# Ezreal11/EaBNet

Hardware: AMD Instinct MI355X
Metric: enhanced frames/sec (16 kHz, 8-mic) at 1/2/4/8 MI355X; RTF per utterance (higher is better)
Workload: dtype f32; 1 GPU; BASELINE configs[1]/[2]: batch of 16 four-second 8-mic 16 kHz utterances per GPU, wave -> STFT+compress -> EaBNet.forward, inference, full hand-written HIP path; batch_per_gpu=16, global_batch=16, mics=8, frames_per_utt=401, freq_bins=161, parallelism=dp1 (independent shards, no collective), pipeline_depth=3

## Files before the change

### eabnet_amd/csrc/conv_gemm.hip

```cpp
#include "device.h"
#include <type_traits>

#define CG_THREADS 256

#define CG_PLAIN 0
#define CG_GLU 1
#define CG_DUAL 2
#define CG_PH2 3
#define CG_XFC 128

#define CG_PMAX 352

template <int MI, int NI, int KU, int MODE, bool PATCH, bool XFT>
struct CgSmem {
    static constexpr int BM = 64 * MI, BN = 64 * NI, LDK = 16 * KU + 4;
    static constexpr int NA = MODE == CG_DUAL ? 2 : 1;
    static constexpr int ATILE = BM * LDK;
    float a[PATCH ? CG_PMAX * LDK : NA * 2 * ATILE];
    float b[2][BN * LDK];
    float xft[2][CG_XFC][2];
    float xsl[2][CG_XFC];
    int dt[EAB_MAX_TAPS];
    int ioff[EAB_MAX_TAPS];
    int last;
    static constexpr int RW = MODE == CG_PH2 ? 2 : 1;
    __attribute__((aligned(16))) unsigned rtab_own[XFT ? BM * RW : 4];
    static_assert(XFT || sizeof(float) * 2 * CG_XFC * 2 >= sizeof(unsigned) * BM * RW, "row table inside xft");
};

__device__ __forceinline__ void cg_merge(float& n, float& mean, float& m2, float nb, float meanb, float m2b) {
    const float nt = n + nb;
    if (nt > 0.0f) {
        const float delta = meanb - mean;
        const float fb = nb / nt;
        mean = fmaf(delta, fb, mean);
        m2 = m2 + m2b + delta * delta * n * fb;
    }
    n = nt;
}

template <int MI, int NI, int KU, int MODE, int XF, bool VEC, int PREC, bool PATCH, bool WIDE = false>
__global__ __launch_bounds__(CG_THREADS, (MI == 2 && NI == 2 && KU == 1 && MODE == CG_GLU) ? 3 : (MODE == CG_PH2 ? 2 : 1)) void conv_gemm_kernel(const eab_conv_desc d) {
    static_assert(MODE != CG_PH2 || (PATCH && NI == 2), "phase-pair form: patch pipeline, one column block per phase and wave");
    static_assert(!PATCH || (KU == 1 && MODE != CG_DUAL && VEC), "patch mode: one unit per stage, single transform");
    constexpr bool H3 = PREC == EAB_PREC_F16X3;
    constexpr bool BF = PREC == EAB_PREC_BF16;
    constexpr bool PH2 = MODE == CG_PH2;
    constexpr bool GLU = MODE != CG_PLAIN;
    constexpr bool DUAL = MODE == CG_DUAL;
    using Smem = CgSmem<MI, NI, KU, MODE, PATCH, XF != EAB_XF_NONE>;
    constexpr int BM = Smem::BM, BN = Smem::BN, LDK = Smem::LDK;
    __shared__ __attribute__((aligned(16))) Smem sm;

    const int tid = threadIdx.x;
    const int lane = tid & 63, wave = tid >> 6;
    const int wm = wave >> 1, wn = wave & 1;
    const int li = lane & 31, lh = lane >> 5;

    const int t_lo = d.win.pos ? *d.win.pos : 0;
    int t_hi = d.win.pos ? (t_lo + d.win.count < d.T ? t_lo + d.win.count : d.T) : d.T;
    const int tiles_per_b = ((d.win.pos ? d.win.count : d.T) * d.No + BM - 1) / BM;
    unsigned vblk = blockIdx.x;
    if (gridDim.x >= 64) {
        const unsigned G = gridDim.x, G8 = G >> 3, rem = G & 7, xcd = vblk & 7, idx = vblk >> 3;
        vblk = xcd * G8 + (xcd < rem ? xcd : rem) + idx;
    }
    const int b = (int)(vblk / (unsigned)tiles_per_b);
    const int tile = (int)vblk - b * tiles_per_b;
    if (d.win.lens) t_hi = min(t_hi, d.win.lens[b]);
    const int Q = t_hi * d.No;
    const int q0 = t_lo * d.No + tile * BM;
    const int n_blk = blockIdx.y * BN;
    const float inv_no = 1.0f / (float)d.No;

#pragma unroll
    for (int j = 0; j < EAB_MAX_TAPS; ++j)
        if (tid == j) {
            sm.dt[j] = d.dt[j];
            sm.ioff[j] = d.ioff[j];
        }

    const int Cout = d.Cout;
    const unsigned row_bytes = (unsigned)(d.Fout * Cout) * 4u, step_bytes = (unsigned)(d.ostride * Cout) * 4u;
    const unsigned phase_bytes = (unsigned)(d.ophase * Cout) * 4u, chan_bytes = (unsigned)Cout * 4u;
    unsigned* const rtab = XF != EAB_XF_NONE ? sm.rtab_own : reinterpret_cast<unsigned*>(&sm.xft[0][0][0]);
    if (tid < BM) {
        const int q = q0 + tid;
        const bool ok = q < Q;
        const int t = eab_div(ok ? q : 0, d.No, inv_no), o = (ok ? q : 0) - t * d.No;
        const unsigned off = ok ? (unsigned)t * row_bytes + (unsigned)o * step_bytes + phase_bytes : EAB_OOB;
        if constexpr (PH2)
            *reinterpret_cast<uint2*>(&rtab[2 * tid]) = make_uint2(off, (ok && 2 * o + 1 < d.Fout) ? off + chan_bytes : EAB_OOB);
        else
            rtab[tid] = off;
    }

    if (XF != EAB_XF_NONE) {
        const int k = tid >> 7, c = tid & (CG_XFC - 1);
        const int Ck = (k == 0 || DUAL) ? d.C0 : d.C1;
        const float* xfk = k == 0 ? d.xf0 : d.xf1;
        const float* slk = k == 0 ? d.slope0 : d.slope1;
        float sc = 1.0f, sh = 0.0f, sl = 1.0f;
        if (c < Ck) {
            if (d.fin_stats && k < d.fin_nsets) {
                const float* gm = k == 0 ? d.fin_gamma0 : d.fin_gamma1;
                const float* bt = k == 0 ? d.fin_beta0 : d.fin_beta1;
                double sn = 0.0, sm = 0.0, sq = 0.0;
                for (int t = 0; t < d.fin_tiles; ++t) {
                    const f32x4 v = *reinterpret_cast<const f32x4*>(
                        &d.fin_stats[((((size_t)b * d.fin_tiles + t) * d.fin_nsets + k) * d.C0 + c) * 4]);
                    const double n = (double)v[0], mu = (double)v[1];
                    sn += n;
                    sm = fma(n, mu, sm);
                    sq += fma(n * mu, mu, (double)v[2]);
                }
                const double mean = sn > 0.0 ? sm / sn : 0.0;
                double var = sn > 0.0 ? sq / sn - mean * mean : 0.0;
                if (var < 0.0) var = 0.0;
                const double scale = (double)gm[c] / sqrt(var + (double)d.fin_eps);
                sc = (float)scale;
                sh = (float)((double)bt[c] - mean * scale);
                sl = slk[c];
            } else if (xfk) {
                const float2 v = *reinterpret_cast<const float2*>(&xfk[((size_t)b * Ck + c) * 2]);
                sc = v.x;
                sh = v.y;
                sl = slk[c];
            }
        }
        sm.xft[k][c][0] = sc;
        sm.xft[k][c][1] = sh;
        sm.xsl[k][c] = sl;
    }

    const int Ctot = d.C0 + d.C1;
    const int UPT = (Ctot + 15) >> 4;
    const int NU = d.ntaps * UPT;
    static_assert(!WIDE || (PREC == EAB_PREC_BF16 && KU == 1 && VEC && !PATCH && XF == EAB_XF_NONE && MODE != CG_DUAL), "WIDE: see above");
    constexpr bool w0 = WIDE, w1 = WIDE;
    const int NS = (w0 || w1) ? d.ntaps * ((w0 ? d.C0 >> 5 : (d.C0 + 15) >> 4) + (d.C1 > 0 ? (w1 ? d.C1 >> 5 : (d.C1 + 15) >> 4) : 0))
                              : (NU + KU - 1) / KU;

    constexpr unsigned esz0 = WIDE ? 2u : 4u, esz1 = WIDE ? 2u : 4u;
    const unsigned bytes0 = (unsigned)d.T * d.Fin * d.C0 * esz0;
    const unsigned bytes1 = (unsigned)d.T * d.Fin * d.C1 * esz1;
    const __amdgpu_buffer_rsrc_t rs0 = __builtin_amdgcn_make_buffer_rsrc(
        const_cast<char*>(reinterpret_cast<const char*>(d.src0)) + (size_t)b * bytes0, 0, bytes0, 0x00020000);
    const __amdgpu_buffer_rsrc_t rs1 = __builtin_amdgcn_make_buffer_rsrc(
        const_cast<char*>(reinterpret_cast<const char*>(d.src1 ? d.src1 : d.src0)) + (d.src1 ? (size_t)b * bytes1 : 0), 0,
        d.src1 ? bytes1 : 0u, 0x00020000);

    const int srow = tid >> 2;
    const int skq = tid & 3;
    const float* wrow[NI];
#pragma unroll
    for (int p = 0; p < NI; ++p) wrow[p] = d.w + (size_t)(n_blk + srow + 64 * p) * d.Kpad + skq * 4;

    f32x16 acc[MI][NI];
#pragma unroll
    for (int mi = 0; mi < MI; ++mi)
#pragma unroll
        for (int ni = 0; ni < NI; ++ni)
#pragma unroll
            for (int r = 0; r < 16; ++r) acc[mi][ni][r] = 0.0f;

    auto lds_barrier = [] { asm volatile("s_waitcnt lgkmcnt(0)\n\ts_barrier" ::: "memory"); };

    __syncthreads();

    if (q0 < Q) {
    if constexpr (PATCH) {
        constexpr int PP = (CG_PMAX + 63) / 64;
        int dt_min = 0, io_min = 0, io_max = 0;
#pragma unroll
        for (int j = 0; j < EAB_MAX_TAPS; ++j)
            if (j < d.ntaps) {
                dt_min = d.dt[j] < dt_min ? d.dt[j] : dt_min;
                io_min = d.ioff[j] < io_min ? d.ioff[j] : io_min;
                io_max = d.ioff[j] > io_max ? d.ioff[j] : io_max;
            }
        const int halo_lo = -io_min;
        const int hi_need = (d.No - 1) * d.istride + io_max - (d.Fin - 1);
        const int Fp = d.Fin + halo_lo + (hi_need > 0 ? hi_need : 0);
        const float inv_fp = 1.0f / (float)Fp;
        const int t_first = eab_div(q0, d.No, inv_no);
        const int t_last = eab_div((q0 + BM < Q ? q0 + BM : (Q > q0 ? Q : q0 + 1)) - 1, d.No, inv_no);
        const int P = (t_last - t_first + 1 - dt_min) * Fp;

        const int d64 = eab_div(64, Fp, inv_fp), m64 = 64 - d64 * Fp;
        int p_tf[PP];
        bool p_ok[PP], p_all[PP];
        {
            const int tr = eab_div(srow, Fp, inv_fp);
            int f = srow - tr * Fp, t_in = t_first + dt_min + tr;
            int tf = t_in * d.Fin + f - halo_lo;
#pragma unroll
            for (int pp = 0; pp < PP; ++pp) {
                p_ok[pp] = p_all[pp] = false;
                p_tf[pp] = 0;
                if (64 * pp < P) {
                    p_ok[pp] = srow + 64 * pp < P && (unsigned)t_in < (unsigned)d.T && (unsigned)(f - halo_lo) < (unsigned)d.Fin;
                    if (XF != EAB_XF_NONE) p_all[pp] = __builtin_amdgcn_ballot_w64(p_ok[pp]) == __builtin_amdgcn_ballot_w64(true);
                    p_tf[pp] = tf;
                    f += m64;
                    t_in += d64;
                    tf += d64 * d.Fin + m64;
                    if (f >= Fp) {
                        f -= Fp;
                        ++t_in;
                        tf += d.Fin - Fp;
                    }
                }
            }
        }
        int fa[MI];
#pragma unroll
        for (int mi = 0; mi < MI; ++mi) {
            int q = q0 + (wm * MI + mi) * 32 + li;
            q = q < Q ? q : (Q > q0 ? Q - 1 : q0);
            const int t = eab_div(q, d.No, inv_no), o = q - t * d.No;
            fa[mi] = ((t - t_first - dt_min) * Fp + o * d.istride + halo_lo) * LDK + 4 * lh;
        }
        const int b_base = (wn * NI * 32 + li) * LDK + 4 * lh;

        f32x4 rp[PP];
        f32x4 rbw0[NI], rbw1[NI];
        int p_tc = 0;
        auto patch_fetch = [&](int chunk) {
            const int c0 = chunk << 4;
            const bool second = (d.C1 > 0) && (c0 >= d.C0);
            const int Cs = second ? d.C1 : d.C0;
            const int c = (second ? c0 - d.C0 : c0) + skq * 4;
            const bool cok = c < Cs;
            p_tc = ((second ? 1 : 0) << 8) | (cok ? c : 0);
#pragma unroll
            for (int pp = 0; pp < PP; ++pp) {
                if (64 * pp >= P) continue;
                const unsigned off = (p_ok[pp] && cok) ? (unsigned)((p_tf[pp] * Cs + c) * 4) : EAB_OOB;
                const u32x4 v = second ? __builtin_amdgcn_raw_buffer_load_b128(rs1, off, 0, 0)
                                       : __builtin_amdgcn_raw_buffer_load_b128(rs0, off, 0, 0);
                rp[pp] = __builtin_bit_cast(f32x4, v);
            }
        };
        auto patch_stash = [&]() {
            f32x4 sh01, sh23, sl;
            if (XF != EAB_XF_NONE) {
                const int cc = p_tc & 0xFF, tb = p_tc >> 8;
                sh01 = *reinterpret_cast<const f32x4*>(&sm.xft[tb][cc][0]);
                sh23 = *reinterpret_cast<const f32x4*>(&sm.xft[tb][cc + 2][0]);
                sl = *reinterpret_cast<const f32x4*>(&sm.xsl[tb][cc]);
            }
#pragma unroll
            for (int pp = 0; pp < PP; ++pp) {
                const int pidx = srow + 64 * pp;
                if (pidx >= CG_PMAX) continue;
                if (64 * pp >= P) continue;
                f32x4 v = rp[pp];
                if (XF != EAB_XF_NONE) {
                    const f32x4 x = eab_xform<XF>(v, sh01, sh23, sl);
                    v = x;
                    if (!p_all[pp]) {
                        asm volatile("; rim" ::: "memory");
                        v = p_ok[pp] ? x : f32x4{0.f, 0.f, 0.f, 0.f};
                    }
                }
                float* arow = &sm.a[pidx * LDK];
                if (BF) {
                    *reinterpret_cast<uint2*>(reinterpret_cast<char*>(arow) + skq * 8) = make_uint2(eab_bf2(v[0], v[1]), eab_bf2(v[2], v[3]));
                } else if (H3) {
                    unsigned h01, l01, h23, l23;
                    eab_split2(v[0], v[1], h01, l01);
                    eab_split2(v[2], v[3], h23, l23);
                    *reinterpret_cast<uint2*>(reinterpret_cast<char*>(arow) + skq * 8) = make_uint2(h01, h23);
                    *reinterpret_cast<uint2*>(reinterpret_cast<char*>(arow) + 32 + skq * 8) = make_uint2(l01, l23);
                } else {
                    *reinterpret_cast<f32x4*>(arow + skq * 4) = v;
                }
            }
        };
        auto b_fetch = [&](int u, f32x4 (&rbw)[NI]) {
            const int uu = u < NU ? u : 0;
#pragma unroll
            for (int p = 0; p < NI; ++p) rbw[p] = *reinterpret_cast<const f32x4*>(wrow[p] + (size_t)uu * 16);
        };
        auto b_stash = [&](int buf, const f32x4 (&rbw)[NI]) {
#pragma unroll
            for (int p = 0; p < NI; ++p) {
                float* brow = &sm.b[buf][(srow + 64 * p) * LDK];
                if (BF) {
                    *reinterpret_cast<uint2*>(reinterpret_cast<char*>(brow) + skq * 8) =
                        make_uint2(eab_bf2(rbw[p][0], rbw[p][1]), eab_bf2(rbw[p][2], rbw[p][3]));
                } else if (H3) {
                    const u32x4 w = __builtin_bit_cast(u32x4, rbw[p]);
                    *reinterpret_cast<uint2*>(reinterpret_cast<char*>(brow) + skq * 8) = make_uint2(w[0], w[1]);
                    *reinterpret_cast<uint2*>(reinterpret_cast<char*>(brow) + 32 + skq * 8) = make_uint2(w[2], w[3]);
                } else {
                    *reinterpret_cast<f32x4*>(brow + skq * 4) = rbw[p];
                }
            }
        };
        auto pcompute_n = [&](int cur, int tap, auto ne_c) {
            constexpr int NE = decltype(ne_c)::value;
            const int toff = (sm.dt[tap] * Fp + sm.ioff[tap]) * LDK;
            if (BF) {
                bf16x8 ab[MI], bb[NE];
#pragma unroll
                for (int mi = 0; mi < MI; ++mi) ab[mi] = *reinterpret_cast<const bf16x8*>(&sm.a[fa[mi] + toff]);
#pragma unroll
                for (int ni = 0; ni < NE; ++ni) bb[ni] = *reinterpret_cast<const bf16x8*>(&sm.b[cur][b_base + ni * 32 * LDK]);
#pragma unroll
                for (int mi = 0; mi < MI; ++mi)
#pragma unroll
                    for (int ni = 0; ni < NE; ++ni)
                        acc[mi][ni] = __builtin_amdgcn_mfma_f32_32x32x16_bf16(ab[mi], bb[ni], acc[mi][ni], 0, 0, 0);
            } else if (H3) {
                h16x8 ah[MI], al[MI], bh[NE], bl[NE];
#pragma unroll
                for (int mi = 0; mi < MI; ++mi) {
                    const char* pa = reinterpret_cast<const char*>(&sm.a[fa[mi] + toff]);
                    ah[mi] = *reinterpret_cast<const h16x8*>(pa);
                    al[mi] = *reinterpret_cast<const h16x8*>(pa + 32);
                }
#pragma unroll
                for (int ni = 0; ni < NE; ++ni) {
                    const char* pb = reinterpret_cast<const char*>(&sm.b[cur][b_base + ni * 32 * LDK]);
                    bh[ni] = *reinterpret_cast<const h16x8*>(pb);
                    bl[ni] = *reinterpret_cast<const h16x8*>(pb + 32);
                }
#pragma unroll
                for (int mi = 0; mi < MI; ++mi)
#pragma unroll
                    for (int ni = 0; ni < NE; ++ni) {
                        acc[mi][ni] = __builtin_amdgcn_mfma_f32_32x32x16_f16(al[mi], bh[ni], acc[mi][ni], 0, 0, 0);
                        acc[mi][ni] = __builtin_amdgcn_mfma_f32_32x32x16_f16(ah[mi], bl[ni], acc[mi][ni], 0, 0, 0);
                        acc[mi][ni] = __builtin_amdgcn_mfma_f32_32x32x16_f16(ah[mi], bh[ni], acc[mi][ni], 0, 0, 0);
                    }
            } else {
#pragma unroll
                for (int g = 0; g < 2; ++g) {
                    f32x4 af[MI], bf[NE];
#pragma unroll
                    for (int mi = 0; mi < MI; ++mi) af[mi] = *reinterpret_cast<const f32x4*>(&sm.a[fa[mi] + toff + g * 8]);
#pragma unroll
                    for (int ni = 0; ni < NE; ++ni)
                        bf[ni] = *reinterpret_cast<const f32x4*>(&sm.b[cur][b_base + ni * 32 * LDK + g * 8]);
#pragma unroll
                    for (int k = 0; k < 4; ++k)
#pragma unroll
                        for (int mi = 0; mi < MI; ++mi)
#pragma unroll
                            for (int ni = 0; ni < NE; ++ni)
                                acc[mi][ni] = __builtin_amdgcn_mfma_f32_32x32x2f32(af[mi][k], bf[ni][k], acc[mi][ni], 0, 0, 0);
                }
            }
        };
        const unsigned p2mask = PH2 ? (unsigned)d.p2_mask1 : ~0u;
        auto pcompute = [&](int cur, int tap) {
            if (PH2 && !((p2mask >> tap) & 1u)) pcompute_n(cur, tap, std::integral_constant<int, 1>{});
            else pcompute_n(cur, tap, std::integral_constant<int, NI>{});
        };

        patch_fetch(0);
        b_fetch(0, rbw0);
        patch_stash();
        b_stash(0, rbw0);
        b_fetch(1, rbw0);
        b_fetch(2, rbw1);
        lds_barrier();
        const int pre = d.ntaps >= 3 ? d.ntaps - 3 : 0;
        int chunk = 0, tap = 0;
        auto stage = [&](int u, int cur, f32x4 (&rnext)[NI]) {
            if (tap == pre && chunk + 1 < UPT) patch_fetch(chunk + 1);
            pcompute(cur, tap);
            if (u + 1 < NU) b_stash(cur ^ 1, rnext);
            b_fetch(u + 3, rnext);
            if (tap == d.ntaps - 1 && chunk + 1 < UPT) {
                lds_barrier();
                patch_stash();
            }
            lds_barrier();
            if (++tap == d.ntaps) { tap = 0; ++chunk; }
        };
        for (int u = 0; u < NU; u += 2) {
            stage(u, 0, rbw0);
            if (u + 1 < NU) stage(u + 1, 1, rbw1);
        }
        __syncthreads();
    } else {
    int a_t[MI], a_f0[MI], a_tf[MI];
    bool a_ok[MI];
#pragma unroll
    for (int p = 0; p < MI; ++p) {
        const int q = q0 + srow + 64 * p;
        a_ok[p] = q < Q;
        const int t = a_ok[p] ? eab_div(q, d.No, inv_no) : 0;
        const int o = a_ok[p] ? q - t * d.No : 0;
        a_t[p] = t;
        a_f0[p] = o * d.istride;
        a_tf[p] = t * d.Fin + o * d.istride;
    }
    struct Stage {
        f32x4 ra[KU][MI], rb[KU][NI];
        f32x4 rb2[BF ? NI : 1];
        int r_tc[KU];
        bool st_ok[KU][MI];
    };
    Stage sa;

    bool tap_ok[MI];
    unsigned tap_b0[MI], tap_b1[MI];
#pragma unroll
    for (int p = 0; p < MI; ++p) {
        tap_ok[p] = false;
        tap_b0[p] = tap_b1[p] = 0u;
    }
    int g_tap = -1, g_c0 = 0, g_w = 16;
    constexpr bool LEAN = KU == 1 && VEC && !DUAL;
    const __amdgpu_buffer_rsrc_t rsw = __builtin_amdgcn_make_buffer_rsrc(const_cast<float*>(d.w), 0, (unsigned)d.N * d.Kpad * 4u, 0x00020000);
// ... 121 lines not shown
                    const int tb = (rg.r_tc[ku] >> 8) & 1, cu = rg.r_tc[ku] & 0xFF;
                    const char* px = reinterpret_cast<const char*>(&sm.xft[0][skq * 4][0]) + (tb * CG_XFC + cu) * 8;
                    const char* ps = reinterpret_cast<const char*>(&sm.xsl[0][skq * 4]) + (tb * CG_XFC + cu) * 4;
                    sh01[0] = *reinterpret_cast<const f32x4*>(px);
                    sh23[0] = *reinterpret_cast<const f32x4*>(px + 16);
                    sl[0] = *reinterpret_cast<const f32x4*>(ps);
                    bool ok_all = true;
#pragma unroll
                    for (int p = 0; p < MI; ++p) ok_all = ok_all && rg.st_ok[ku][p];
                    all_ok = __builtin_amdgcn_ballot_w64(ok_all) == __builtin_amdgcn_ballot_w64(true);
                } else {
                const int cc = rg.r_tc[ku] & 0xFF;
#pragma unroll
                for (int k = 0; k < (DUAL ? 2 : 1); ++k) {
                    const int tb = DUAL ? k : (rg.r_tc[ku] >> 8);
                    sh01[k] = *reinterpret_cast<const f32x4*>(&sm.xft[tb][cc][0]);
                    sh23[k] = *reinterpret_cast<const f32x4*>(&sm.xft[tb][cc + 2][0]);
                    sl[k] = *reinterpret_cast<const f32x4*>(&sm.xsl[tb][cc]);
                }
                }
            }
#pragma unroll
            for (int p = 0; p < MI; ++p) {
#pragma unroll
                for (int k = 0; k < (DUAL ? 2 : 1); ++k) {
                    f32x4 v = rg.ra[ku][p];
                    if (XF != EAB_XF_NONE) {
                        v = eab_xform<XF>(v, sh01[k], sh23[k], sl[k]);
                        if (!all_ok) {
                            asm volatile("; rim" ::: "memory");
                            v = rg.st_ok[ku][p] ? v : f32x4{0.f, 0.f, 0.f, 0.f};
                        }
                    }
                    float* arow = &sm.a[(k * 2 + buf) * Smem::ATILE + (srow + 64 * p) * LDK + ku * 16];
                    if (BF) {
                        constexpr bool half = WIDE;
                        if (half)
                            *reinterpret_cast<u32x4*>(reinterpret_cast<char*>(arow) + skq * 16) = __builtin_bit_cast(u32x4, v);
                        else
                            *reinterpret_cast<uint2*>(reinterpret_cast<char*>(arow) + skq * 8) = make_uint2(eab_bf2(v[0], v[1]), eab_bf2(v[2], v[3]));
                    } else if (H3) {
                        unsigned h01, l01, h23, l23;
                        eab_split2(v[0], v[1], h01, l01);
                        eab_split2(v[2], v[3], h23, l23);
                        *reinterpret_cast<uint2*>(reinterpret_cast<char*>(arow) + skq * 8) = make_uint2(h01, h23);
                        *reinterpret_cast<uint2*>(reinterpret_cast<char*>(arow) + 32 + skq * 8) = make_uint2(l01, l23);
                    } else {
                        *reinterpret_cast<f32x4*>(arow + skq * 4) = v;
                    }
                }
            }
#pragma unroll
            for (int p = 0; p < NI; ++p) {
                float* brow = &sm.b[buf][(srow + 64 * p) * LDK + ku * 16];
                if (BF) {
                    if constexpr (WIDE) {
                        const f32x4 r0 = rg.rb[ku][p], r1 = rg.rb2[BF ? p : 0];
                        *reinterpret_cast<u32x4*>(reinterpret_cast<char*>(brow) + skq * 16) =
                            u32x4{eab_bf2(r0[0], r0[1]), eab_bf2(r0[2], r0[3]), eab_bf2(r1[0], r1[1]), eab_bf2(r1[2], r1[3])};
                    } else {
                        *reinterpret_cast<uint2*>(reinterpret_cast<char*>(brow) + skq * 8) =
                            make_uint2(eab_bf2(rg.rb[ku][p][0], rg.rb[ku][p][1]), eab_bf2(rg.rb[ku][p][2], rg.rb[ku][p][3]));
                    }
                } else if (H3) {
                    const u32x4 w = __builtin_bit_cast(u32x4, rg.rb[ku][p]);
                    *reinterpret_cast<uint2*>(reinterpret_cast<char*>(brow) + skq * 8) = make_uint2(w[0], w[1]);
                    *reinterpret_cast<uint2*>(reinterpret_cast<char*>(brow) + 32 + skq * 8) = make_uint2(w[2], w[3]);
                } else {
                    *reinterpret_cast<f32x4*>(brow + skq * 4) = rg.rb[ku][p];
                }
            }
        }
    };

    fetch(0, sa);
    stash(0, sa);
    lds_barrier();

    const int a_base = (wm * MI * 32 + li) * LDK + 4 * lh;
    const int b_base = (wn * NI * 32 + li) * LDK + 4 * lh;

    auto compute = [&](int cur) {
        if (BF) {
#pragma unroll
            for (int ku = 0; ku < KU; ++ku) {
                bf16x8 ab[Smem::NA][MI], bb[NI];
#pragma unroll
                for (int k = 0; k < Smem::NA; ++k)
#pragma unroll
                    for (int mi = 0; mi < MI; ++mi)
                        ab[k][mi] = *reinterpret_cast<const bf16x8*>(&sm.a[(k * 2 + cur) * Smem::ATILE + a_base + mi * 32 * LDK + ku * 16]);
#pragma unroll
                for (int ni = 0; ni < NI; ++ni) bb[ni] = *reinterpret_cast<const bf16x8*>(&sm.b[cur][b_base + ni * 32 * LDK + ku * 16]);
#pragma unroll
                for (int mi = 0; mi < MI; ++mi)
#pragma unroll
                    for (int ni = 0; ni < NI; ++ni)
                        acc[mi][ni] = __builtin_amdgcn_mfma_f32_32x32x16_bf16(ab[DUAL ? ni : 0][mi], bb[ni], acc[mi][ni], 0, 0, 0);
            }
            if constexpr (WIDE) {
                bf16x8 ab[MI], bb[NI];
#pragma unroll
                for (int mi = 0; mi < MI; ++mi) ab[mi] = *reinterpret_cast<const bf16x8*>(&sm.a[cur * Smem::ATILE + a_base + mi * 32 * LDK + 8]);
#pragma unroll
                for (int ni = 0; ni < NI; ++ni) bb[ni] = *reinterpret_cast<const bf16x8*>(&sm.b[cur][b_base + ni * 32 * LDK + 8]);
#pragma unroll
                for (int mi = 0; mi < MI; ++mi)
#pragma unroll
                    for (int ni = 0; ni < NI; ++ni)
                        acc[mi][ni] = __builtin_amdgcn_mfma_f32_32x32x16_bf16(ab[mi], bb[ni], acc[mi][ni], 0, 0, 0);
            }
        } else if (H3) {
#pragma unroll
            for (int ku = 0; ku < KU; ++ku) {
                h16x8 ah[Smem::NA][MI], al[Smem::NA][MI], bh[NI], bl[NI];
#pragma unroll
                for (int k = 0; k < Smem::NA; ++k)
#pragma unroll
                    for (int mi = 0; mi < MI; ++mi) {
                        const char* pa = reinterpret_cast<const char*>(&sm.a[(k * 2 + cur) * Smem::ATILE + a_base + mi * 32 * LDK + ku * 16]);
                        ah[k][mi] = *reinterpret_cast<const h16x8*>(pa);
                        al[k][mi] = *reinterpret_cast<const h16x8*>(pa + 32);
                    }
#pragma unroll
                for (int ni = 0; ni < NI; ++ni) {
                    const char* pb = reinterpret_cast<const char*>(&sm.b[cur][b_base + ni * 32 * LDK + ku * 16]);
                    bh[ni] = *reinterpret_cast<const h16x8*>(pb);
                    bl[ni] = *reinterpret_cast<const h16x8*>(pb + 32);
                }
#pragma unroll
                for (int mi = 0; mi < MI; ++mi)
#pragma unroll
                    for (int ni = 0; ni < NI; ++ni) {
                        const int ka = DUAL ? ni : 0;
                        acc[mi][ni] = __builtin_amdgcn_mfma_f32_32x32x16_f16(al[ka][mi], bh[ni], acc[mi][ni], 0, 0, 0);
                        acc[mi][ni] = __builtin_amdgcn_mfma_f32_32x32x16_f16(ah[ka][mi], bl[ni], acc[mi][ni], 0, 0, 0);
                        acc[mi][ni] = __builtin_amdgcn_mfma_f32_32x32x16_f16(ah[ka][mi], bh[ni], acc[mi][ni], 0, 0, 0);
                    }
            }
        } else {
#pragma unroll
        for (int g = 0; g < 2 * KU; ++g) {
            f32x4 af[Smem::NA][MI], bf[NI];
#pragma unroll
            for (int k = 0; k < Smem::NA; ++k)
#pragma unroll
                for (int mi = 0; mi < MI; ++mi)
                    af[k][mi] = *reinterpret_cast<const f32x4*>(&sm.a[(k * 2 + cur) * Smem::ATILE + a_base + mi * 32 * LDK + g * 8]);
#pragma unroll
            for (int ni = 0; ni < NI; ++ni)
                bf[ni] = *reinterpret_cast<const f32x4*>(&sm.b[cur][b_base + ni * 32 * LDK + g * 8]);
#pragma unroll
            for (int k = 0; k < 4; ++k)
#pragma unroll
                for (int mi = 0; mi < MI; ++mi)
#pragma unroll
                    for (int ni = 0; ni < NI; ++ni)
                        acc[mi][ni] = __builtin_amdgcn_mfma_f32_32x32x2f32(af[DUAL ? ni : 0][mi][k], bf[ni][k],
                                                                           acc[mi][ni], 0, 0, 0);
        }
        }
    };
    constexpr bool PF2 = MI * NI <= 2 && KU == 1 && MODE == CG_PLAIN;
    if constexpr (PF2) {
        Stage sb;
        if (NS > 1) fetch(1, sb);
        for (int s = 0; s < NS; s += 2) {
            if (s + 2 < NS) fetch(s + 2, sa);
            compute(0);
            if (s + 1 < NS) stash(1, sb);
            lds_barrier();
            if (s + 1 < NS) {
                if (s + 3 < NS) fetch(s + 3, sb);
                compute(1);
                if (s + 2 < NS) stash(0, sa);
                lds_barrier();
            }
        }
    } else {
    for (int s = 0; s < NS; ++s) {
        const int cur = s & 1;
// ... 210 lines not shown
                    }
                } else {
                    v = acc[mi][c][r] + bias_v[c];
                }
                if (d.epi == EAB_EPI_RELU) v = fmaxf(v, 0.0f);
                else if (d.epi == EAB_EPI_MULSIG) v = auxv[r][c] * eab_fast_sigmoid(v);
                else if (d.epi == EAB_EPI_ADD) v = v + auxv[r][c];
                const unsigned o4 = off[r] + 4u * ch[c];
                __builtin_amdgcn_raw_buffer_store_b32(__builtin_bit_cast(unsigned, v), r_dst, o4, 0, 0);
                if (d.dst_acc)
                    __builtin_amdgcn_raw_buffer_store_b32(__builtin_bit_cast(unsigned, v + accv[r][c]), r_acc, o4, 0, 0);
                if (rowok[r]) {
                    const bool first = scount == 0.0f;
                    const float g0 = eab_prelu(v, st_slope[0][c]);
                    if (first) skk[0][c] = g0;
                    const float e0 = g0 - skk[0][c];
                    ssum[0][c] += e0;
                    ssq[0][c] = fmaf(e0, e0, ssq[0][c]);
                    if (two_sets) {
                        const float g1 = eab_prelu(v, st_slope[1][c]);
                        if (first) skk[1][c] = g1;
                        const float e1 = g1 - skk[1][c];
                        ssum[1][c] += e1;
                        ssq[1][c] = fmaf(e1, e1, ssq[1][c]);
                    }
                }
            }
            if (rowok[r]) scount += 1.0f;
        }
    }

    }
    if (d.stats) {
        float* red = &sm.a[0];
        float mean[2][NC], m2[2][NC];
        float cnt = scount;
        const float inv_n = scount > 0.0f ? 1.0f / scount : 0.0f;
#pragma unroll
        for (int s = 0; s < 2; ++s)
#pragma unroll
            for (int c = 0; c < NC; ++c) {
                mean[s][c] = fmaf(ssum[s][c], inv_n, skk[s][c]);
                m2[s][c] = fmaxf(ssq[s][c] - ssum[s][c] * ssum[s][c] * inv_n, 0.0f);
            }
        const float cnt_o = __shfl_xor(cnt, 32);
#pragma unroll
        for (int s = 0; s < 2; ++s)
#pragma unroll
            for (int c = 0; c < NC; ++c) {
                float n = cnt;
                const float mo = __shfl_xor(mean[s][c], 32), qo = __shfl_xor(m2[s][c], 32);
                if (lh == 0) cg_merge(n, mean[s][c], m2[s][c], cnt_o, mo, qo);
            }
        cnt += cnt_o;
        if (lh == 0) {
#pragma unroll
            for (int s = 0; s < 2; ++s)
#pragma unroll
                for (int c = 0; c < NC; ++c) {
                    const int i = ((((wm * 2 + wn) * 2 + s) * NC + c) * 32 + li) * 3;
                    red[i] = cnt;
                    red[i + 1] = mean[s][c];
                    red[i + 2] = m2[s][c];
                }
        }
        __syncthreads();
        if (wm == 0 && lh == 0) {
            const size_t tbase = ((size_t)b * d.stat_tiles + d.stat_tile0 + tile) * d.nsets;
#pragma unroll
            for (int s = 0; s < 2; ++s) {
                if (s >= d.nsets) break;
#pragma unroll
                for (int c = 0; c < NC; ++c) {
                    const int i0 = ((((0 * 2 + wn) * 2 + s) * NC + c) * 32 + li) * 3;
                    const int i1 = ((((1 * 2 + wn) * 2 + s) * NC + c) * 32 + li) * 3;
                    float n = red[i0], mu = red[i0 + 1], q = red[i0 + 2];
                    cg_merge(n, mu, q, red[i1], red[i1 + 1], red[i1 + 2]);
                    *reinterpret_cast<f32x4*>(&d.stats[((tbase + s) * Cout + ch[c]) * 4]) = f32x4{n, mu, q, 0.0f};
                }
            }
        }
        if (d.fz_counter) {
            __threadfence();
            __syncthreads();
            if (tid == 0) sm.last = atomicAdd(&d.fz_counter[b], 1) == d.stat_tiles - 1;
            __syncthreads();
            if (sm.last) {
                __threadfence();
                const int nch = d.nsets * Cout;
                const int NSL = CG_THREADS / nch;
                const int e = tid % nch, slice = tid / nch;
                const int s = e / Cout, c = e - s * Cout;
                double* dred = reinterpret_cast<double*>(&sm.a[0]);
                double sn = 0.0, sm_ = 0.0, sq = 0.0;
                if (slice < NSL) {
                    const float* p = d.stats + (((size_t)b * d.stat_tiles) * d.nsets + s) * Cout * 4 + (size_t)c * 4;
                    const size_t stride = (size_t)d.nsets * Cout * 4;
                    for (int t = slice; t < d.stat_tiles; t += NSL) {
                        const f32x4 v = *reinterpret_cast<const f32x4*>(p + (size_t)t * stride);
                        const double n = (double)v[0], mu = (double)v[1];
                        sn += n;
                        sm_ = fma(n, mu, sm_);
                        sq += fma(n * mu, mu, (double)v[2]);
                    }
                    dred[(0 * NSL + slice) * nch + e] = sn;
                    dred[(1 * NSL + slice) * nch + e] = sm_;
                    dred[(2 * NSL + slice) * nch + e] = sq;
                }
                __syncthreads();
                if (slice == 0) {
                    sn = sm_ = sq = 0.0;
                    for (int k = 0; k < NSL; ++k) {
                        sn += dred[(0 * NSL + k) * nch + e];
                        sm_ += dred[(1 * NSL + k) * nch + e];
                        sq += dred[(2 * NSL + k) * nch + e];
                    }
                    const double mean = sn > 0.0 ? sm_ / sn : 0.0;
                    double var = sn > 0.0 ? sq / sn - mean * mean : 0.0;
                    if (var < 0.0) var = 0.0;
                    const float* gm = s == 0 ? d.fz_gamma0 : d.fz_gamma1;
                    const float* bt = s == 0 ? d.fz_beta0 : d.fz_beta1;
                    float* xf = s == 0 ? d.fz_xf0 : d.fz_xf1;
                    const double scale = (double)gm[c] / sqrt(var + (double)d.fz_eps);
                    *reinterpret_cast<float2*>(&xf[((size_t)b * Cout + c) * 2]) = make_float2((float)scale, (float)((double)bt[c] - mean * scale));
                }
                if (tid == 0) d.fz_counter[b] = 0;
// ... 2 lines not shown
    }
}

extern "C" int eab_conv_tiles(int T, int No, int bm) {
    if (T <= 0 || No <= 0 || (bm != 16 && bm != 32 && bm != 64 && bm != 128)) return -1;
    long long q = (long long)T * No;
    return (int)((q + bm - 1) / bm);
}

int eab_conv_st(const eab_conv_desc* d, hipStream_t s);

template <int MI, int NI, int KU, int MODE, int XF, bool VEC>
static int cg_launch(const eab_conv_desc* d, hipStream_t s) {
    constexpr int BM = 64 * MI, BN = 64 * NI;
    const int tiles = eab_conv_tiles(d->win.pos ? d->win.count : d->T, d->No, BM);
    dim3 grid((unsigned)(d->B * tiles), (unsigned)(d->N / BN));
    constexpr bool can_patch = KU == 1 && MODE != CG_DUAL && VEC && XF != EAB_XF_PRELU_NORM;
    if (d->korder == EAB_KORDER_CHUNK) {
        if constexpr (can_patch) {
            if (d->precision == EAB_PREC_F16X3)
                hipLaunchKernelGGL((conv_gemm_kernel<MI, NI, 1, MODE, XF, true, EAB_PREC_F16X3, true>), grid,
                                   dim3(CG_THREADS), 0, s, *d);
            else if (d->precision == EAB_PREC_BF16)
                hipLaunchKernelGGL((conv_gemm_kernel<MI, NI, 1, MODE, XF, true, EAB_PREC_BF16, true>), grid,
                                   dim3(CG_THREADS), 0, s, *d);
            else
                hipLaunchKernelGGL((conv_gemm_kernel<MI, NI, 1, MODE, XF, true, EAB_PREC_F32, true>), grid,
                                   dim3(CG_THREADS), 0, s, *d);
            EAB_RETURN_LAUNCH_STATUS();
        } else {
            return EAB_EUNSUPPORTED;
        }
    }
    if constexpr (MODE == CG_PH2) {
        return EAB_EUNSUPPORTED;
    } else {
    if (d->precision == EAB_PREC_F16X3) {
        if constexpr (VEC)
            hipLaunchKernelGGL((conv_gemm_kernel<MI, NI, KU, MODE, XF, VEC, EAB_PREC_F16X3, false>), grid,
                               dim3(CG_THREADS), 0, s, *d);
        else
            return EAB_EUNSUPPORTED;
    } else if (d->precision == EAB_PREC_BF16) {
        if constexpr (VEC) {
            if (d->src_bf16) {
                if constexpr (KU == 1 && XF == EAB_XF_NONE && MODE != CG_DUAL)
                    hipLaunchKernelGGL((conv_gemm_kernel<MI, NI, KU, MODE, XF, VEC, EAB_PREC_BF16, false, true>), grid,
                                       dim3(CG_THREADS), 0, s, *d);
                else
                    return EAB_EUNSUPPORTED;
            } else {
                hipLaunchKernelGGL((conv_gemm_kernel<MI, NI, KU, MODE, XF, VEC, EAB_PREC_BF16, false>), grid,
                                   dim3(CG_THREADS), 0, s, *d);
            }
        } else {
            return EAB_EUNSUPPORTED;
        }
    } else {
        hipLaunchKernelGGL((conv_gemm_kernel<MI, NI, KU, MODE, XF, VEC, EAB_PREC_F32, false>), grid, dim3(CG_THREADS), 0,
                           s, *d);
    }
    EAB_RETURN_LAUNCH_STATUS();
    }
}

static long long cg_patch_positions(const eab_conv_desc* d) {
    int dt_min = 0, io_min = 0, io_max = 0;
// ... 81 lines not shown
        EAB_CHECK_ARG(fin || (d->xf0 == nullptr) == (d->slope0 == nullptr));
        EAB_CHECK_ARG(fin || dual || (d->xf1 == nullptr) == (d->slope1 == nullptr));
    }
    if (dual) {
        EAB_CHECK_ARG(d->C1 == 0 && d->xf_mode != EAB_XF_NONE && d->slope0 && d->slope1);
        EAB_CHECK_ARG(fin || (d->xf0 && d->xf1));
    }
    EAB_CHECK_ARG((d->epi != EAB_EPI_MULSIG && d->epi != EAB_EPI_ADD) || d->aux);
    EAB_CHECK_ARG(d->nsets >= 0 && d->nsets <= 2 && (d->nsets == 0) == (d->stats == nullptr));
    EAB_CHECK_ARG(d->korder == EAB_KORDER_FRAG ? (d->bm == 16 || d->bm == 32 || d->bm == 64) : (d->bm == 64 || d->bm == 128));
    if (d->fz_counter) {
        EAB_CHECK_ARG(d->stats && d->nsets >= 1 && d->nsets * d->Cout <= CG_THREADS && d->win.pos == nullptr);
        EAB_CHECK_ARG(d->fz_gamma0 && d->fz_beta0 && d->fz_xf0 && (d->nsets == 1 || (d->fz_gamma1 && d->fz_beta1 && d->fz_xf1)));
    }
    if (d->stats) {
        const int tiles = eab_conv_tiles(d->T, d->No, d->bm) + (d->ph1_No > 0 ? eab_conv_tiles(d->T, d->ph1_No, d->bm) : 0);
        EAB_CHECK_ARG(d->stat_tile0 >= 0 && d->stat_tile0 + tiles <= d->stat_tiles);
    }
    EAB_CHECK_ARG((long long)d->B * (eab_conv_tiles(d->T, d->No, d->bm) + (d->ph1_No > 0 ? eab_conv_tiles(d->T, d->ph1_No, d->bm) : 0)) < (1ll << 31));
    hipStream_t s = eab_stream(stream);
    if (d->korder == EAB_KORDER_FRAG) return eab_conv_st(d, s);
    const int mi = d->bm / 64;
    const bool vec = (d->C0 % 4 == 0) && (d->C1 % 4 == 0);
    const bool has_xf = d->xf_mode != EAB_XF_NONE && (d->xf0 || d->xf1 || fin);
    const int xf = has_xf ? d->xf_mode : EAB_XF_NONE;
    if (xf != EAB_XF_NONE)
        EAB_CHECK_ARG(d->C0 <= CG_XFC && d->C1 <= CG_XFC && vec);
    int ku = (mi == 1 && !glu && vec && d->Fin == 1) ? 4 : 1;
    if (d->korder == EAB_KORDER_CHUNK) ku = 1;
    if (ku == 4 && !(mi == 1 && !glu && vec)) ku = 1;
    if (ku == 2 && (!vec || dual)) ku = 1;
    if (ph2) {
        if (!vec || xf == EAB_XF_PRELU_NORM) return EAB_EUNSUPPORTED;
        if (xf == EAB_XF_NORM_PRELU)
            return mi == 2 ? cg_launch<2, 2, 1, CG_PH2, EAB_XF_NORM_PRELU, true>(d, s) : cg_launch<1, 2, 1, CG_PH2, EAB_XF_NORM_PRELU, true>(d, s);
        return mi == 2 ? cg_launch<2, 2, 1, CG_PH2, EAB_XF_NONE, true>(d, s) : cg_launch<1, 2, 1, CG_PH2, EAB_XF_NONE, true>(d, s);
    }
    if (dual) {
        if (d->N != 128 || mi != 1 || xf != EAB_XF_PRELU_NORM) return EAB_EUNSUPPORTED;
        return cg_pick_ku<1, 2, CG_DUAL, EAB_XF_PRELU_NORM, true>(d, s, ku == 2 ? 1 : ku);
    }
    if (glu) {
        if (d->N % 128 != 0 || xf == EAB_XF_PRELU_NORM) return EAB_EUNSUPPORTED;
        if (!vec) return mi == 2 ? cg_pick_ku<2, 2, CG_GLU, 0, false>(d, s, 1) : cg_pick_ku<1, 2, CG_GLU, 0, false>(d, s, 1);
        if (xf == EAB_XF_NORM_PRELU)
            return mi == 2 ? cg_pick_ku<2, 2, CG_GLU, EAB_XF_NORM_PRELU, true>(d, s, ku)
                           : cg_pick_ku<1, 2, CG_GLU, EAB_XF_NORM_PRELU, true>(d, s, ku);
        return mi == 2 ? cg_pick_ku<2, 2, CG_GLU, 0, true>(d, s, ku) : cg_pick_ku<1, 2, CG_GLU, 0, true>(d, s, ku);
    }
    if (!vec) return EAB_EUNSUPPORTED;
#define CG_DISPATCH_XF(MI_, NI_)                                                           \
    (xf == EAB_XF_NONE        ? cg_pick_ku<MI_, NI_, CG_PLAIN, EAB_XF_NONE, true>(d, s, ku) \
     : xf == EAB_XF_NORM_PRELU ? cg_pick_ku<MI_, NI_, CG_PLAIN, EAB_XF_NORM_PRELU, true>(d, s, ku) \
                               : cg_pick_ku<MI_, NI_, CG_PLAIN, EAB_XF_PRELU_NORM, true>(d, s, ku))
    if (d->N % 128 == 0) return mi == 2 ? CG_DISPATCH_XF(2, 2) : CG_DISPATCH_XF(1, 2);
    if (d->N % 64 == 0) return mi == 2 ? CG_DISPATCH_XF(2, 1) : CG_DISPATCH_XF(1, 1);
#undef CG_DISPATCH_XF
    return EAB_EUNSUPPORTED;
}

extern "C" int eab_conv_bf16(const eab_conv_desc* d, eab_stream_t stream) {
    EAB_CHECK_ARG(d);
    eab_conv_desc dd = *d;
    dd.precision = EAB_PREC_BF16;
    return eab_conv_f32(&dd, stream);
}
// ... 1 lines not shown
```

Before: 997,500 frames/s.

## Double-buffer patch tile in phase-pair conv GEMM for two-tap layers

Adds a second LDS patch buffer for the phase-pair (PH2) patch pipeline. When a layer has exactly two taps, the next channel chunk is fetched and stashed into the alternate buffer while the current one is consumed, which removes the extra barrier that previously sat before each patch restash. It also defers building the norm/PReLU transform tables until after the first global loads are issued, so their latency overlaps. Other tap counts, or EAB_PATCH_BUFS=1, fall back to a single-buffer PH2S variant. The cost is doubled patch LDS, which is held under a static assert so two workgroups still fit per CU.

```diff
diff --git a/eabnet_amd/csrc/conv_gemm.hip b/eabnet_amd/csrc/conv_gemm.hip
--- a/eabnet_amd/csrc/conv_gemm.hip
+++ b/eabnet_amd/csrc/conv_gemm.hip
@@ -1,4 +1,5 @@
 #include "device.h"
+#include <cstdlib>
 #include <type_traits>
 
 #define CG_THREADS 256
@@ -7,23 +8,26 @@
 #define CG_GLU 1
 #define CG_DUAL 2
 #define CG_PH2 3
+#define CG_PH2S 4
 #define CG_XFC 128
 
 #define CG_PMAX 352
+#define CG_LDS_CU 163840
 
 template <int MI, int NI, int KU, int MODE, bool PATCH, bool XFT>
 struct CgSmem {
     static constexpr int BM = 64 * MI, BN = 64 * NI, LDK = 16 * KU + 4;
     static constexpr int NA = MODE == CG_DUAL ? 2 : 1;
     static constexpr int ATILE = BM * LDK;
-    float a[PATCH ? CG_PMAX * LDK : NA * 2 * ATILE];
+    static constexpr int PBUF = (PATCH && MODE == CG_PH2) ? 2 : 1;
+    float a[PBUF][PATCH ? CG_PMAX * LDK : NA * 2 * ATILE];
     float b[2][BN * LDK];
     float xft[2][CG_XFC][2];
     float xsl[2][CG_XFC];
     int dt[EAB_MAX_TAPS];
     int ioff[EAB_MAX_TAPS];
     int last;
-    static constexpr int RW = MODE == CG_PH2 ? 2 : 1;
+    static constexpr int RW = (MODE == CG_PH2 || MODE == CG_PH2S) ? 2 : 1;
     __attribute__((aligned(16))) unsigned rtab_own[XFT ? BM * RW : 4];
     static_assert(XFT || sizeof(float) * 2 * CG_XFC * 2 >= sizeof(unsigned) * BM * RW, "row table inside xft");
 };
@@ -39,17 +43,62 @@
     n = nt;
 }
 
+#define CG_XF_TABLES()                                                                                                         \
+    if (XF != EAB_XF_NONE) {                                                                                                   \
+                                          \
+                                           \
+                                             \
+                                                                \
+        const int k = tid >> 7, c = tid & (CG_XFC - 1);                                                                        \
+        const int Ck = (k == 0 || DUAL) ? d.C0 : d.C1;                                                                         \
+        const float* xfk = k == 0 ? d.xf0 : d.xf1;                                                                             \
+        const float* slk = k == 0 ? d.slope0 : d.slope1;                                                                       \
+        float sc = 1.0f, sh = 0.0f, sl = 1.0f;                                                                                 \
+        if (c < Ck) {                                                                                                          \
+            if (d.fin_stats && k < d.fin_nsets) {                                                                              \
+                const float* gm = k == 0 ? d.fin_gamma0 : d.fin_gamma1;                                                        \
+                const float* bt = k == 0 ? d.fin_beta0 : d.fin_beta1;                                                          \
+                double sn = 0.0, sm = 0.0, sq = 0.0;                               \
+                for (int t = 0; t < d.fin_tiles; ++t) {                                                                        \
+                    const f32x4 v = *reinterpret_cast<const f32x4*>(                                                           \
+                        &d.fin_stats[((((size_t)b * d.fin_tiles + t) * d.fin_nsets + k) * d.C0 + c) * 4]);                     \
+                    const double n = (double)v[0], mu = (double)v[1];                                                          \
+                    sn += n;                                                                                                   \
+                    sm = fma(n, mu, sm);                                                                                       \
+                    sq += fma(n * mu, mu, (double)v[2]);                                                                       \
+                }                                                                                                              \
+                const double mean = sn > 0.0 ? sm / sn : 0.0;                                                                  \
+                double var = sn > 0.0 ? sq / sn - mean * mean : 0.0;                                                           \
+                if (var < 0.0) var = 0.0;                                                                                      \
+                const double scale = (double)gm[c] / sqrt(var + (double)d.fin_eps);                                            \
+                sc = (float)scale;                                                                                             \
+                sh = (float)((double)bt[c] - mean * scale);                                                                    \
+                sl = slk[c];                                                                                                   \
+            } else if (xfk) {                                                                                                  \
+                const float2 v = *reinterpret_cast<const float2*>(&xfk[((size_t)b * Ck + c) * 2]);                             \
+                sc = v.x;                                                                                                      \
+                sh = v.y;                                                                                                      \
+                sl = slk[c];                                                                                                   \
+            }                                                                                                                  \
+        }                                                                                                                      \
+        sm.xft[k][c][0] = sc;                                                                                                  \
+        sm.xft[k][c][1] = sh;                                                                                                  \
+        sm.xsl[k][c] = sl;                                                                                                     \
+    }
+
 template <int MI, int NI, int KU, int MODE, int XF, bool VEC, int PREC, bool PATCH, bool WIDE = false>
-__global__ __launch_bounds__(CG_THREADS, (MI == 2 && NI == 2 && KU == 1 && MODE == CG_GLU) ? 3 : (MODE == CG_PH2 ? 2 : 1)) void conv_gemm_kernel(const eab_conv_desc d) {
-    static_assert(MODE != CG_PH2 || (PATCH && NI == 2), "phase-pair form: patch pipeline, one column block per phase and wave");
+__global__ __launch_bounds__(CG_THREADS, (MI == 2 && NI == 2 && KU == 1 && MODE == CG_GLU) ? 3 : ((MODE == CG_PH2 || MODE == CG_PH2S) ? 2 : 1)) void conv_gemm_kernel(const eab_conv_desc d) {
+    constexpr bool PH2 = MODE == CG_PH2 || MODE == CG_PH2S;
+    static_assert(!PH2 || (PATCH && NI == 2), "phase-pair form: patch pipeline, one column block per phase and wave");
     static_assert(!PATCH || (KU == 1 && MODE != CG_DUAL && VEC), "patch mode: one unit per stage, single transform");
     constexpr bool H3 = PREC == EAB_PREC_F16X3;
     constexpr bool BF = PREC == EAB_PREC_BF16;
-    constexpr bool PH2 = MODE == CG_PH2;
     constexpr bool GLU = MODE != CG_PLAIN;
     constexpr bool DUAL = MODE == CG_DUAL;
     using Smem = CgSmem<MI, NI, KU, MODE, PATCH, XF != EAB_XF_NONE>;
     constexpr int BM = Smem::BM, BN = Smem::BN, LDK = Smem::LDK;
+    constexpr int PBUF = Smem::PBUF;
+    static_assert(PBUF == 1 || 2 * sizeof(Smem) <= CG_LDS_CU, "two patch buffers: two workgroups must still share a CU's LDS");
     __shared__ __attribute__((aligned(16))) Smem sm;
 
     const int tid = threadIdx.x;
@@ -95,43 +144,8 @@
             rtab[tid] = off;
     }
 
-    if (XF != EAB_XF_NONE) {
-        const int k = tid >> 7, c = tid & (CG_XFC - 1);
-        const int Ck = (k == 0 || DUAL) ? d.C0 : d.C1;
-        const float* xfk = k == 0 ? d.xf0 : d.xf1;
-        const float* slk = k == 0 ? d.slope0 : d.slope1;
-        float sc = 1.0f, sh = 0.0f, sl = 1.0f;
-        if (c < Ck) {
-            if (d.fin_stats && k < d.fin_nsets) {
-                const float* gm = k == 0 ? d.fin_gamma0 : d.fin_gamma1;
-                const float* bt = k == 0 ? d.fin_beta0 : d.fin_beta1;
-                double sn = 0.0, sm = 0.0, sq = 0.0;
-                for (int t = 0; t < d.fin_tiles; ++t) {
-                    const f32x4 v = *reinterpret_cast<const f32x4*>(
-                        &d.fin_stats[((((size_t)b * d.fin_tiles + t) * d.fin_nsets + k) * d.C0 + c) * 4]);
-                    const double n = (double)v[0], mu = (double)v[1];
-                    sn += n;
-                    sm = fma(n, mu, sm);
-                    sq += fma(n * mu, mu, (double)v[2]);
-                }
-                const double mean = sn > 0.0 ? sm / sn : 0.0;
-                double var = sn > 0.0 ? sq / sn - mean * mean : 0.0;
-                if (var < 0.0) var = 0.0;
-                const double scale = (double)gm[c] / sqrt(var + (double)d.fin_eps);
-                sc = (float)scale;
-                sh = (float)((double)bt[c] - mean * scale);
-                sl = slk[c];
-            } else if (xfk) {
-                const float2 v = *reinterpret_cast<const float2*>(&xfk[((size_t)b * Ck + c) * 2]);
-                sc = v.x;
-                sh = v.y;
-                sl = slk[c];
-            }
-        }
-        sm.xft[k][c][0] = sc;
-        sm.xft[k][c][1] = sh;
-        sm.xsl[k][c] = sl;
-    }
+    constexpr bool EARLY = PATCH && XF != EAB_XF_NONE;
+    if constexpr (!EARLY) { CG_XF_TABLES() }
 
     const int Ctot = d.C0 + d.C1;
     const int UPT = (Ctot + 15) >> 4;
@@ -166,8 +180,12 @@
 
     auto lds_barrier = [] { asm volatile("s_waitcnt lgkmcnt(0)\n\ts_barrier" ::: "memory"); };
 
-    __syncthreads();
-
+    if constexpr (!EARLY) __syncthreads();
+
+    if (EARLY && q0 >= Q) {
+        CG_XF_TABLES()
+        __syncthreads();
+    }
     if (q0 < Q) {
     if constexpr (PATCH) {
         constexpr int PP = (CG_PMAX + 63) / 64;
@@ -226,23 +244,24 @@
         f32x4 rp[PP];
         f32x4 rbw0[NI], rbw1[NI];
         int p_tc = 0;
-        auto patch_fetch = [&](int chunk) {
+        auto patch_fetch = [&](int chunk, auto all_c) {
+            constexpr bool ALL = decltype(all_c)::value;
             const int c0 = chunk << 4;
             const bool second = (d.C1 > 0) && (c0 >= d.C0);
             const int Cs = second ? d.C1 : d.C0;
             const int c = (second ? c0 - d.C0 : c0) + skq * 4;
-            const bool cok = c < Cs;
+            const bool cok = ALL ? (c < Cs && chunk < UPT) : c < Cs;
             p_tc = ((second ? 1 : 0) << 8) | (cok ? c : 0);
 #pragma unroll
             for (int pp = 0; pp < PP; ++pp) {
-                if (64 * pp >= P) continue;
+                if (!ALL && 64 * pp >= P) continue;
                 const unsigned off = (p_ok[pp] && cok) ? (unsigned)((p_tf[pp] * Cs + c) * 4) : EAB_OOB;
                 const u32x4 v = second ? __builtin_amdgcn_raw_buffer_load_b128(rs1, off, 0, 0)
                                        : __builtin_amdgcn_raw_buffer_load_b128(rs0, off, 0, 0);
                 rp[pp] = __builtin_bit_cast(f32x4, v);
             }
         };
-        auto patch_stash = [&]() {
+        auto patch_stash = [&](int pb) {
             f32x4 sh01, sh23, sl;
             if (XF != EAB_XF_NONE) {
                 const int cc = p_tc & 0xFF, tb = p_tc >> 8;
@@ -264,7 +283,7 @@
                         v = p_ok[pp] ? x : f32x4{0.f, 0.f, 0.f, 0.f};
                     }
                 }
-                float* arow = &sm.a[pidx * LDK];
+                float* arow = &sm.a[pb][pidx * LDK];
                 if (BF) {
                     *reinterpret_cast<uint2*>(reinterpret_cast<char*>(arow) + skq * 8) = make_uint2(eab_bf2(v[0], v[1]), eab_bf2(v[2], v[3]));
                 } else if (H3) {
@@ -299,13 +318,14 @@
                 }
             }
         };
-        auto pcompute_n = [&](int cur, int tap, auto ne_c) {
+        auto pcompute_n = [&](int cur, int tap, int pb, auto ne_c) {
             constexpr int NE = decltype(ne_c)::value;
             const int toff = (sm.dt[tap] * Fp + sm.ioff[tap]) * LDK;
+            const float* const pa0 = sm.a[pb];
             if (BF) {
                 bf16x8 ab[MI], bb[NE];
 #pragma unroll
-                for (int mi = 0; mi < MI; ++mi) ab[mi] = *reinterpret_cast<const bf16x8*>(&sm.a[fa[mi] + toff]);
+                for (int mi = 0; mi < MI; ++mi) ab[mi] = *reinterpret_cast<const bf16x8*>(&pa0[fa[mi] + toff]);
 #pragma unroll
                 for (int ni = 0; ni < NE; ++ni) bb[ni] = *reinterpret_cast<const bf16x8*>(&sm.b[cur][b_base + ni * 32 * LDK]);
 #pragma unroll
@@ -317,7 +337,7 @@
                 h16x8 ah[MI], al[MI], bh[NE], bl[NE];
 #pragma unroll
                 for (int mi = 0; mi < MI; ++mi) {
-                    const char* pa = reinterpret_cast<const char*>(&sm.a[fa[mi] + toff]);
+                    const char* pa = reinterpret_cast<const char*>(&pa0[fa[mi] + toff]);
                     ah[mi] = *reinterpret_cast<const h16x8*>(pa);
                     al[mi] = *reinterpret_cast<const h16x8*>(pa + 32);
                 }
@@ -340,7 +360,7 @@
                 for (int g = 0; g < 2; ++g) {
                     f32x4 af[MI], bf[NE];
 #pragma unroll
-                    for (int mi = 0; mi < MI; ++mi) af[mi] = *reinterpret_cast<const f32x4*>(&sm.a[fa[mi] + toff + g * 8]);
+                    for (int mi = 0; mi < MI; ++mi) af[mi] = *reinterpret_cast<const f32x4*>(&pa0[fa[mi] + toff + g * 8]);
 #pragma unroll
                     for (int ni = 0; ni < NE; ++ni)
                         bf[ni] = *reinterpret_cast<const f32x4*>(&sm.b[cur][b_base + ni * 32 * LDK + g * 8]);
@@ -355,28 +375,51 @@
             }
         };
         const unsigned p2mask = PH2 ? (unsigned)d.p2_mask1 : ~0u;
-        auto pcompute = [&](int cur, int tap) {
-            if (PH2 && !((p2mask >> tap) & 1u)) pcompute_n(cur, tap, std::integral_constant<int, 1>{});
-            else pcompute_n(cur, tap, std::integral_constant<int, NI>{});
+        auto pcompute = [&](int cur, int tap, int pb) {
+            if (PH2 && !((p2mask >> tap) & 1u)) pcompute_n(cur, tap, pb, std::integral_constant<int, 1>{});
+            else pcompute_n(cur, tap, pb, std::integral_constant<int, NI>{});
         };
 
-        patch_fetch(0);
+        patch_fetch(0, std::false_type{});
         b_fetch(0, rbw0);
-        patch_stash();
+        if constexpr (EARLY) {
+            CG_XF_TABLES()
+            __syncthreads();
+        }
+        patch_stash(0);
         b_stash(0, rbw0);
+        if constexpr (PBUF == 2) {
+            patch_fetch(1, std::true_type{});
+            b_fetch(1, rbw0);
+            b_fetch(2, rbw1);
+            lds_barrier();
+            for (int c = 0; c < UPT; ++c) {
+                const int u = 2 * c, pb = c & 1;
+                pcompute(0, 0, pb);
+                if (c + 1 < UPT) patch_stash(pb ^ 1);
+                b_stash(1, rbw0);
+                patch_fetch(c + 2, std::true_type{});
+                b_fetch(u + 3, rbw0);
+                lds_barrier();
+                pcompute(1, 1, pb);
+                if (c + 1 < UPT) b_stash(0, rbw1);
+                b_fetch(u + 4, rbw1);
+                lds_barrier();
+            }
+        } else {
         b_fetch(1, rbw0);
         b_fetch(2, rbw1);
         lds_barrier();
         const int pre = d.ntaps >= 3 ? d.ntaps - 3 : 0;
         int chunk = 0, tap = 0;
         auto stage = [&](int u, int cur, f32x4 (&rnext)[NI]) {
-            if (tap == pre && chunk + 1 < UPT) patch_fetch(chunk + 1);
-            pcompute(cur, tap);
+            if (tap == pre && chunk + 1 < UPT) patch_fetch(chunk + 1, std::false_type{});
+            pcompute(cur, tap, 0);
             if (u + 1 < NU) b_stash(cur ^ 1, rnext);
             b_fetch(u + 3, rnext);
             if (tap == d.ntaps - 1 && chunk + 1 < UPT) {
                 lds_barrier();
-                patch_stash();
+                patch_stash(0);
             }
             lds_barrier();
             if (++tap == d.ntaps) { tap = 0; ++chunk; }
@@ -384,6 +427,7 @@
         for (int u = 0; u < NU; u += 2) {
             stage(u, 0, rbw0);
             if (u + 1 < NU) stage(u + 1, 1, rbw1);
+        }
         }
         __syncthreads();
     } else {
@@ -571,7 +615,7 @@
                             v = rg.st_ok[ku][p] ? v : f32x4{0.f, 0.f, 0.f, 0.f};
                         }
                     }
-                    float* arow = &sm.a[(k * 2 + buf) * Smem::ATILE + (srow + 64 * p) * LDK + ku * 16];
+                    float* arow = &sm.a[0][(k * 2 + buf) * Smem::ATILE + (srow + 64 * p) * LDK + ku * 16];
                     if (BF) {
                         constexpr bool half = WIDE;
                         if (half)
@@ -628,7 +672,7 @@
                 for (int k = 0; k < Smem::NA; ++k)
 #pragma unroll
                     for (int mi = 0; mi < MI; ++mi)
-                        ab[k][mi] = *reinterpret_cast<const bf16x8*>(&sm.a[(k * 2 + cur) * Smem::ATILE + a_base + mi * 32 * LDK + ku * 16]);
+                        ab[k][mi] = *reinterpret_cast<const bf16x8*>(&sm.a[0][(k * 2 + cur) * Smem::ATILE + a_base + mi * 32 * LDK + ku * 16]);
 #pragma unroll
                 for (int ni = 0; ni < NI; ++ni) bb[ni] = *reinterpret_cast<const bf16x8*>(&sm.b[cur][b_base + ni * 32 * LDK + ku * 16]);
 #pragma unroll
@@ -640,7 +684,7 @@
             if constexpr (WIDE) {
                 bf16x8 ab[MI], bb[NI];
 #pragma unroll
-                for (int mi = 0; mi < MI; ++mi) ab[mi] = *reinterpret_cast<const bf16x8*>(&sm.a[cur * Smem::ATILE + a_base + mi * 32 * LDK + 8]);
+                for (int mi = 0; mi < MI; ++mi) ab[mi] = *reinterpret_cast<const bf16x8*>(&sm.a[0][cur * Smem::ATILE + a_base + mi * 32 * LDK + 8]);
 #pragma unroll
                 for (int ni = 0; ni < NI; ++ni) bb[ni] = *reinterpret_cast<const bf16x8*>(&sm.b[cur][b_base + ni * 32 * LDK + 8]);
 #pragma unroll
@@ -657,7 +701,7 @@
                 for (int k = 0; k < Smem::NA; ++k)
 #pragma unroll
                     for (int mi = 0; mi < MI; ++mi) {
-                        const char* pa = reinterpret_cast<const char*>(&sm.a[(k * 2 + cur) * Smem::ATILE + a_base + mi * 32 * LDK + ku * 16]);
+                        const char* pa = reinterpret_cast<const char*>(&sm.a[0][(k * 2 + cur) * Smem::ATILE + a_base + mi * 32 * LDK + ku * 16]);
                         ah[k][mi] = *reinterpret_cast<const h16x8*>(pa);
                         al[k][mi] = *reinterpret_cast<const h16x8*>(pa + 32);
                     }
@@ -685,7 +729,7 @@
             for (int k = 0; k < Smem::NA; ++k)
 #pragma unroll
                 for (int mi = 0; mi < MI; ++mi)
-                    af[k][mi] = *reinterpret_cast<const f32x4*>(&sm.a[(k * 2 + cur) * Smem::ATILE + a_base + mi * 32 * LDK + g * 8]);
+                    af[k][mi] = *reinterpret_cast<const f32x4*>(&sm.a[0][(k * 2 + cur) * Smem::ATILE + a_base + mi * 32 * LDK + g * 8]);
 #pragma unroll
             for (int ni = 0; ni < NI; ++ni)
                 bf[ni] = *reinterpret_cast<const f32x4*>(&sm.b[cur][b_base + ni * 32 * LDK + g * 8]);
@@ -962,7 +1006,7 @@
 
     }
     if (d.stats) {
-        float* red = &sm.a[0];
+        float* red = &sm.a[0][0];
         float mean[2][NC], m2[2][NC];
         float cnt = scount;
         const float inv_n = scount > 0.0f ? 1.0f / scount : 0.0f;
@@ -1021,7 +1065,7 @@
                 const int NSL = CG_THREADS / nch;
                 const int e = tid % nch, slice = tid / nch;
                 const int s = e / Cout, c = e - s * Cout;
-                double* dred = reinterpret_cast<double*>(&sm.a[0]);
+                double* dred = reinterpret_cast<double*>(&sm.a[0][0]);
                 double sn = 0.0, sm_ = 0.0, sq = 0.0;
                 if (slice < NSL) {
                     const float* p = d.stats + (((size_t)b * d.stat_tiles) * d.nsets + s) * Cout * 4 + (size_t)c * 4;
@@ -1090,7 +1134,7 @@
             return EAB_EUNSUPPORTED;
         }
     }
-    if constexpr (MODE == CG_PH2) {
+    if constexpr (MODE == CG_PH2 || MODE == CG_PH2S) {
         return EAB_EUNSUPPORTED;
     } else {
     if (d->precision == EAB_PREC_F16X3) {
@@ -1238,6 +1282,12 @@
     if (ku == 2 && (!vec || dual)) ku = 1;
     if (ph2) {
         if (!vec || xf == EAB_XF_PRELU_NORM) return EAB_EUNSUPPORTED;
+        const char* pbufs = getenv("EAB_PATCH_BUFS");
+        if (d->ntaps != 2 || (pbufs && pbufs[0] == '1' && pbufs[1] == '\0')) {
+            if (xf == EAB_XF_NORM_PRELU)
+                return mi == 2 ? cg_launch<2, 2, 1, CG_PH2S, EAB_XF_NORM_PRELU, true>(d, s) : cg_launch<1, 2, 1, CG_PH2S, EAB_XF_NORM_PRELU, true>(d, s);
+            return mi == 2 ? cg_launch<2, 2, 1, CG_PH2S, EAB_XF_NONE, true>(d, s) : cg_launch<1, 2, 1, CG_PH2S, EAB_XF_NONE, true>(d, s);
+        }
         if (xf == EAB_XF_NORM_PRELU)
             return mi == 2 ? cg_launch<2, 2, 1, CG_PH2, EAB_XF_NORM_PRELU, true>(d, s) : cg_launch<1, 2, 1, CG_PH2, EAB_XF_NORM_PRELU, true>(d, s);
         return mi == 2 ? cg_launch<2, 2, 1, CG_PH2, EAB_XF_NONE, true>(d, s) : cg_launch<1, 2, 1, CG_PH2, EAB_XF_NONE, true>(d, s);
```

After: 994,100 frames/s. Within noise of the previous version (-0.3%).
